# arpitbansal297/Cold-Diffusion-Models

Hardware: AMD Instinct MI355X
Metric: unet_train_imgs_per_sec (higher is better)
Workload: dtype f32 storage/accumulate; dense-conv GEMM operands bf16x3; 1 GPU; CelebA-128 denoising cold diffusion (BASELINE config 3): Unet(dim=64,(1,2,4,8),ch=3) @128x128, T=200, optimizer step = 2 micro-batches x 32 img (one fused forward / backward pass over all of them: same draws, same gradient sum) + Adam + EMA/10; per_gpu_batch=32, gradient_accumulate_every=2, parallelism=single

## Files before the change

cold-diffusion-models_amd/csrc/cdf_common.h:

```cpp
#pragma once
#include <stdint.h>
#include <stddef.h>

#ifdef CDF_EMU
#include "hipemu.h"
#else
#include <hip/hip_runtime.h>
#define CDF_LAUNCH(kernel, grid, block, shmem, stream, ...) \
    hipLaunchKernelGGL(kernel, grid, block, shmem, stream, __VA_ARGS__)
#define CDF_DYN_SMEM(name) extern __shared__ __attribute__((aligned(16))) unsigned char name[]
#define CDF_LDS_BARRIER() asm volatile("s_waitcnt lgkmcnt(0)\n\ts_barrier" ::: "memory")
#define CDF_GLDS16(gptr, lds_base)                                                                            \
    __builtin_amdgcn_global_load_lds((const __attribute__((address_space(1))) void*)(gptr),                    \
                                     (__attribute__((address_space(3))) void*)(lds_base), 16, 0, 0)
#define CDF_WAIT_DMA() asm volatile("s_waitcnt vmcnt(0)" ::: "memory")
#define CDF_WAIT_DMA_LEAVE(N) asm volatile("s_waitcnt vmcnt(%0)" ::"n"(N) : "memory")
#define CDF_SCHED_FENCE() __builtin_amdgcn_sched_barrier(0)
#define CDF_WAIT_LDS() __builtin_amdgcn_s_waitcnt(0xC07F)
typedef float f32x4_t __attribute__((ext_vector_type(4)));
typedef float f32x16_t __attribute__((ext_vector_type(16)));
#endif
#ifndef CDF_EMU
struct CdfDeviceLatch {
    unsigned long long seen = 0;
// ... 78 lines not shown
#ifdef CDF_EMU
struct cdf_buf { const char* base; unsigned bytes; };
static inline cdf_buf cdf_make_buf(const void* p, unsigned bytes) { return cdf_buf{(const char*)p, bytes}; }
static inline float4 cdf_buf_ld(const cdf_buf& b, unsigned off, const float4*) {
    float4 v = make_float4(0.f, 0.f, 0.f, 0.f);
    if ((unsigned long long)off + 16 <= b.bytes) v = *(const float4*)(b.base + off);
    return v;
}
static inline uint2 cdf_buf_ld(const cdf_buf& b, unsigned off, const uint2*) {
    uint2 v = make_uint2(0u, 0u);
    if ((unsigned long long)off + 8 <= b.bytes) v = *(const uint2*)(b.base + off);
    return v;
}
static inline void cdf_buf_st(const cdf_buf& b, unsigned off, const float4& v) {
    if ((unsigned long long)off + 16 <= b.bytes) *(float4*)(b.base + off) = v;
}
static inline void cdf_buf_st(const cdf_buf& b, unsigned off, const uint2& v) {
    if ((unsigned long long)off + 8 <= b.bytes) *(uint2*)(b.base + off) = v;
}
#else
typedef __amdgpu_buffer_rsrc_t cdf_buf;
__device__ __forceinline__ cdf_buf cdf_make_buf(const void* p, unsigned bytes) {
    return __builtin_amdgcn_make_buffer_rsrc((void*)p, 0, (int)bytes, 0x00020000);
}
__device__ __forceinline__ float4 cdf_buf_ld(const cdf_buf& b, unsigned off, const float4*) {
    typedef int i4_t __attribute__((ext_vector_type(4)));
    const i4_t v = __builtin_amdgcn_raw_buffer_load_b128(b, (int)off, 0, 0);
    return make_float4(__int_as_float(v[0]), __int_as_float(v[1]), __int_as_float(v[2]), __int_as_float(v[3]));
}
__device__ __forceinline__ uint2 cdf_buf_ld(const cdf_buf& b, unsigned off, const uint2*) {
    typedef int i2_t __attribute__((ext_vector_type(2)));
    const i2_t v = __builtin_amdgcn_raw_buffer_load_b64(b, (int)off, 0, 0);
    return make_uint2((unsigned)v[0], (unsigned)v[1]);
}
__device__ __forceinline__ void cdf_buf_st(const cdf_buf& b, unsigned off, const float4& v) {
    typedef int i4_t __attribute__((ext_vector_type(4)));
    const i4_t t = {__float_as_int(v.x), __float_as_int(v.y), __float_as_int(v.z), __float_as_int(v.w)};
    __builtin_amdgcn_raw_buffer_store_b128(t, b, (int)off, 0, 0);
}
__device__ __forceinline__ void cdf_buf_st(const cdf_buf& b, unsigned off, const uint2& v) {
    typedef int i2_t __attribute__((ext_vector_type(2)));
    const i2_t t = {(int)v.x, (int)v.y};
    __builtin_amdgcn_raw_buffer_store_b64(t, b, (int)off, 0, 0);
}
#endif
__device__ __forceinline__ float4 cdf_quad_raw(const float4& v, const float4*) { return v; }
__device__ __forceinline__ uint2 cdf_quad_raw(const float4& v, const uint2*) { return make_uint2(cdf_pack2bf(v.x, v.y), cdf_pack2bf(v.z, v.w)); }
__device__ __forceinline__ void cdf_ld4_bf(float* v, const void* base, long long off) {
    const float4 t = cdf_quad_cvt(*(const uint2*)((const unsigned short*)base + off));
    v[0] = t.x; v[1] = t.y; v[2] = t.z; v[3] = t.w;
}
__device__ __forceinline__ void cdf_st4_bf(void* base, long long off, const float* v) {
    uint2 h;
    h.x = cdf_pack2bf(v[0], v[1]);
    h.y = cdf_pack2bf(v[2], v[3]);
    *(uint2*)((unsigned short*)base + off) = h;
}
#define CDF_IO_RES_BF16 1
#define CDF_IO_PRE_BF16 2
#define CDF_IO_MUL_BF16 4
#define CDF_IO_PRE_GRAD 8

#define CDF_OK 0
#define CDF_E_INVALID (-1)
#define CDF_E_UNSUPPORTED (-2)
#define CDF_E_LAUNCH (-3)

#define CDF_WAVE 64
#define CDF_S ((hipStream_t)stream)

void cdf_set_error(const char* fmt, ...);
int cdf_check_launch(const char* what);

#define CDF_REQUIRE(cond, ...)                  \
    do {                                        \
        if (!(cond)) {                          \
            cdf_set_error(__VA_ARGS__);         \
            return CDF_E_INVALID;               \
        }                                       \
    } while (0)

static inline int cdf_cdiv(long long a, long long b) { return (int)((a + b - 1) / b); }

__device__ __forceinline__ int cdf_xcd_order(int bid, int nblk) {
    const int q = nblk >> 3, r = nblk & 7;
    const int xcd = bid & 7, idx = bid >> 3;
    const int base = xcd < r ? xcd * (q + 1) : r * (q + 1) + (xcd - r) * q;
    return base + idx;
}

__device__ __forceinline__ float cdf_wave_sum(float v) {
#pragma unroll
    for (int o = 32; o > 0; o >>= 1) v += __shfl_xor(v, o);
    return v;
}
__device__ __forceinline__ float cdf_wave_max(float v) {
#pragma unroll
    for (int o = 32; o > 0; o >>= 1) v = fmaxf(v, __shfl_xor(v, o));
    return v;
}
__device__ __forceinline__ float cdf_group_sum(float v, int width) {
    for (int o = width >> 1; o > 0; o >>= 1) v += __shfl_xor(v, o);
    return v;
}

__device__ __forceinline__ unsigned cdf_hash32(unsigned long long seed, unsigned long long idx) {
    unsigned long long z = seed + idx * 0x9E3779B97F4A7C15ull;
    z = (z ^ (z >> 30)) * 0xBF58476D1CE4E5B9ull;
    z = (z ^ (z >> 27)) * 0x94D049BB133111EBull;
    z = z ^ (z >> 31);
    return (unsigned)(z >> 32);
}

__device__ __forceinline__ float cdf_erf_fast(float z, float& ez2) {
    const float az = fabsf(z);
#ifdef CDF_EMU
    const float t = 1.0f / fmaf(0.3275911f, az, 1.0f);
    ez2 = expf(-az * az);
#else
    const float t = __builtin_amdgcn_rcpf(fmaf(0.3275911f, az, 1.0f));
    ez2 = __expf(-az * az);
#endif
    float p = fmaf(1.061405429f, t, -1.453152027f);
    p = fmaf(p, t, 1.421413741f);
    p = fmaf(p, t, -0.284496736f);
    p = fmaf(p, t, 0.254829592f);
    const float r = fmaf(-p * t, ez2, 1.0f);
    return copysignf(r, z);
}
__device__ __forceinline__ float cdf_gelu(float x) {
    float e;
    return 0.5f * x * (1.0f + cdf_erf_fast(x * 0.70710678118654752440f, e));
}
__device__ __forceinline__ float cdf_gelu_grad(float x) {
    float e;
    const float cdf = 0.5f * (1.0f + cdf_erf_fast(x * 0.70710678118654752440f, e));
    return cdf + x * (0.39894228040143267794f * e);
}
__device__ __forceinline__ float cdf_gelu_both(float x, float& grad) {
    float e;
    const float er = cdf_erf_fast(x * 0.70710678118654752440f, e);
    const float cdf = 0.5f * (1.0f + er);
    grad = cdf + x * (0.39894228040143267794f * e);
    return 0.5f * x * (1.0f + er);
}
__device__ __forceinline__ float cdf_sigmoid(float x) { return 1.0f / (1.0f + expf(-x)); }
__device__ __forceinline__ float cdf_silu(float x) { return x * cdf_sigmoid(x); }
__device__ __forceinline__ float cdf_silu_grad(float x) {
    const float s = cdf_sigmoid(x);
    return s * (1.0f + x * (1.0f - s));
}
```

cold-diffusion-models_amd/csrc/cdf_conv_sp.h:

```cpp
#pragma once
#include "cdf_common.h"
#include "cdf_epilogue.h"
#include "colddiff.h"

#define CDF_MAX_TAPS 16

typedef short bf16x8_v __attribute__((ext_vector_type(8)));
typedef short bf16x4_v __attribute__((ext_vector_type(4)));
typedef unsigned u32x4_v __attribute__((ext_vector_type(4)));
#ifdef CDF_EMU
#define CDF_MFMA_BF16(a, b, c) __builtin_amdgcn_mfma_f32_32x32x16_bf16(a, b, c, 0, 0, 0)
static inline bf16x4_v cdf_lds_read_tr16(const unsigned short* p) { return hipemu::ds_read_tr16_b64(p); }
#else
typedef __bf16 bf16x8_hw __attribute__((ext_vector_type(8)));
#define CDF_MFMA_BF16(a, b, c) \
    __builtin_amdgcn_mfma_f32_32x32x16_bf16(__builtin_bit_cast(bf16x8_hw, a), __builtin_bit_cast(bf16x8_hw, b), c, 0, 0, 0)
__device__ __forceinline__ bf16x4_v cdf_lds_read_tr16(const unsigned short* p) {
    return __builtin_amdgcn_ds_read_tr16_b64_v4i16((__attribute__((address_space(3))) bf16x4_v*)p);
}
#endif

struct SpPhase {
    int oy, ox, ntaps;
    signed char dy[CDF_MAX_TAPS], dx[CDF_MAX_TAPS], wi[CDF_MAX_TAPS];
// ... 130 lines not shown
        bx = v % gx;
        const int t2 = v / gx;
        by = t2 % gy;
        bz = t2 / gy;
    }
}

#define CDF_GLDS16_K(g, l) CDF_GLDS16(g, l)

struct SpxArgs {
    const unsigned short* x_hi;
    const unsigned short* x_lo;
    const unsigned short* zero;
    const unsigned short* w_hi;
    const unsigned short* w_lo;
    float* y;
    const float* bias;
    const float* sbias;
    const float* res;
    float* pre;
    const float* mul;
    int ldx, ldk, ldy, ld_sbias, ldr, ldp, ldm;
    int B, H, W, Cin, OH, OW, Cout, QH, QW, os, is;
    int act, mul_mode, accumulate, nphase, vec;
    int taprot;
    int dephase;
    unsigned short* ys_hi;
    unsigned short* ys_lo;
    int ld_ys;
    int ksplit;
    float* ks_ws;
    int ks_ld;
    int io_bf;
    int epi;
    const float* ln_x;
    const float* ln_mean;
    const float* ln_rstd;
    float* ln_part;
    int ld_lnx;
    SpPhase ph[4];
};

struct RawEpiArgs {
    int Cout, vec, os, QH, QW, OH, OW, ldy, ldp, ldm, ldr, ld_sbias, ld_ys, act, mul_mode, accumulate, io_bf;
    const float* bias;
    const float* sbias;
    float* pre;
    const float* mul;
    const float* res;
    unsigned short* ys_hi;
    unsigned short* ys_lo;
};

struct SpxWgradArgs {
    const unsigned short* a_hi;
    const unsigned short* a_lo;
    const unsigned short* b_hi;
    const unsigned short* b_lo;
    const unsigned short* zero;
    float* out;
    float* bsum;
    int lda, ldb, ldo;
    int B, QH, QW;
    int HA, WA, sa, HB, WB, sb;
    int CA, CB;
    int ntaps, nsplit, m_per_split, xcd_swizzle;
    signed char day[CDF_MAX_TAPS], dax[CDF_MAX_TAPS], dby[CDF_MAX_TAPS], dbx[CDF_MAX_TAPS];
};

static const cdf_gemm_tuning kTuneDefault = {(int)sizeof(cdf_gemm_tuning), 0, 0, 0, 1, 1, 1, 47, 1, 0, 1, 1, 1, 1, 1, 0, 1};
static inline const cdf_gemm_tuning* cdf_tune(const cdf_gemm_tuning* t) { return (t && t->size == (int)sizeof(cdf_gemm_tuning)) ? t : &kTuneDefault; }
static inline bool cdf_tune_ok(const cdf_gemm_tuning* t) {
    if (!t) return true;
    const bool bm_ok = t->tile_bm == 0 || t->tile_bm == 64 || t->tile_bm == 128 || (t->tile_bm == 256 && (t->tile_bn == 0 || t->tile_bn == 128));
    const bool bn_ok = t->tile_bn == 0 || t->tile_bn == 64 || t->tile_bn == 128;
    return t->size == (int)sizeof(cdf_gemm_tuning) && bm_ok && bn_ok && (t->max_bm == 0 || t->max_bm == 128 || t->max_bm == 256) &&
           (t->halo_bm == 0 || t->halo_bm == 128 || t->halo_bm == 256) && t->halo >= 0 && t->halo <= 127 && t->halo_min_tiles >= 0 && t->resident_reserve >= 0 && t->resident_reserve <= 248 && (t->rowhalo_stream == 0 || t->rowhalo_stream == 1) && (t->epilogue == 0 || t->epilogue == 1);
}
#define CDF_TUNE_CHECK(t, who)                                                                                                          \
    CDF_REQUIRE(cdf_tune_ok(t), who ": bad cdf_gemm_tuning (size %d, expected %d; tile_bm 0/64/128/256 (256 with tile_bn 0/128), tile_bn 0/64/128, " \
                                    "max_bm 0/128/256, halo_bm 0/128/256, halo 0..127, rowhalo_stream 0/1, resident_reserve 0..248, epilogue 0/1): start from cdf_gemm_tuning_default",            \
                (t) ? (t)->size : 0, (int)sizeof(cdf_gemm_tuning))

static inline int cdf_num_cus() {
#ifdef CDF_EMU
    return 8;
#else
    static int n[64] = {0};
    int dev = 0;
    if (hipGetDevice(&dev) != hipSuccess || dev < 0 || dev >= 64) return 256;
    if (!n[dev]) {
        int cus = 0;
        n[dev] = (hipDeviceGetAttribute(&cus, hipDeviceAttributeMultiprocessorCount, dev) == hipSuccess && cus >= 8) ? cus / 8 * 8 : 256;
    }
    return n[dev];
#endif
}


struct CdfPlan {
    int code, tiles, grid;
};
enum { CDF_FORM_ROWHALO = 1, CDF_FORM_HALO = 2, CDF_FORM_SPX = 3, CDF_FORM_WGRAD_ROW3 = 1, CDF_FORM_WGRAD_SPX = 2, CDF_FORM_WGRAD_STACK2 = 3 };
static inline int cdf_plan_set(CdfPlan* p, int form, int bm, int bn, int stages, int ksplit, int w, long long tiles, long long grid) {
    p->code = form << 24 | (bm / 64) << 20 | (bn / 64) << 16 | stages << 12 | ksplit << 4 | (w / 16);
    p->tiles = (int)tiles;
    p->grid = (int)grid;
    return CDF_OK;
}

int cdf_launch_igemm_halo(int ns, int W, bool n64, int bm, const SpxArgs& a, int M, hipStream_t s, CdfPlan* plan = nullptr);
int cdf_launch_igemm_rowhalo(int ns, int W, bool n64, const SpxArgs& a, int M, hipStream_t s, int reserve, CdfPlan* plan = nullptr);
```

cold-diffusion-models_amd/csrc/k_conv.hip:

```cpp
#include <atomic>
#include "cdf_common.h"
#include "cdf_epilogue.h"
#include "colddiff.h"

#define CDF_MAX_TAPS 16

struct ConvPhase {
    int oy, ox, ntaps;
    signed char dy[CDF_MAX_TAPS], dx[CDF_MAX_TAPS], wi[CDF_MAX_TAPS];
};

struct ConvArgs {
    const float* x;
    const float* w;
    float* y;
    const float* bias;
    const float* sbias;
    const float* res;
    float* pre;
    const float* mul;
    int ldx, ldw, ldy, ld_sbias, ldr, ldp, ldm;
    int B, H, W, Cin, OH, OW, Cout, QH, QW, os, is;
    int act;
    int mul_mode;
    int accumulate;
    int nphase, vec;
    unsigned short* ys_hi;
    unsigned short* ys_lo;
    int ld_ys;
    int io_bf;
    long long x_bs, w_bs, y_bs;
    long long x_bs2, w_bs2, y_bs2;
    int epi_follow;
    int batch2;
    ConvPhase ph[4];
};

__device__ __forceinline__ int cdf_xcd_swizzle(int bid, int nblk) {
    const int q = nblk >> 3, r = nblk & 7;
    const int xcd = bid & 7, idx = bid >> 3;
    const int base = xcd < r ? xcd * (q + 1) : r * (q + 1) + (xcd - r) * q;
    return base + idx;
}

template <int BM, int BN, int WM, int WN, bool BT>
__global__ void __launch_bounds__(256, 4) conv_igemm_kernel(ConvArgs a) {
    constexpr int BK = 16, AS = BK + 4;
    constexpr int MT = WM / 32, NT = WN / 32, WAVES_N = BN / WN;
    constexpr int APASS = BM / 64;
    constexpr int BVEC = BK * BN / 4;
    constexpr int BPASS = (BVEC + 255) / 256;
    static_assert((BM / WM) * (BN / WN) == 4, "4 waves per block");
    constexpr int ASZ = BM * AS, BSZ = BK * BN;
    constexpr int EPI_ROWS = (BM / WM) * 32, EPI_SZ = EPI_ROWS * (BN + 8);
    constexpr int SMEM = 2 * (ASZ + BSZ) > EPI_SZ ? 2 * (ASZ + BSZ) : EPI_SZ;
    __shared__ __attribute__((aligned(16))) float smem[SMEM];
    float (*As)[ASZ] = (float (*)[ASZ])smem;
    float (*Bs)[BSZ] = (float (*)[BSZ])(smem + 2 * ASZ);

    const int tid = threadIdx.x, lane = tid & 63, wave = tid >> 6;
    const int wm = wave / WAVES_N, wn = wave % WAVES_N;
    const int M = a.B * a.QH * a.QW;
    const int tiles_n = (a.Cout + BN - 1) / BN, tiles_m = (M + BM - 1) / BM;
    const int tile = cdf_xcd_swizzle(blockIdx.x, tiles_m * tiles_n);
    const int tile_m = tile / tiles_n, tile_n = tile - tile_m * tiles_n;
    const ConvPhase& ph = a.ph[blockIdx.y];
    const int zo = blockIdx.z / a.batch2, zi = blockIdx.z - zo * a.batch2;
    const float* X = a.x + (long long)zo * a.x_bs + (long long)zi * a.x_bs2;
    const float* Wt = a.w + (long long)zo * a.w_bs + (long long)zi * a.w_bs2;
    float* Y = a.y + (long long)zo * a.y_bs + (long long)zi * a.y_bs2;
    long long pix_off = 0;
    if (a.epi_follow) {
        pix_off = ((long long)zo * a.y_bs + (long long)zi * a.y_bs2) / a.ldy;
        Y = a.y;
    }

    const int a_col = (tid & 3) * 4;
    int a_iy0[APASS], a_ix0[APASS];
    unsigned a_pix[APASS];
#pragma unroll
    for (int p = 0; p < APASS; ++p) {
        const int m = tile_m * BM + (tid >> 2) + 64 * p;
        if (m < M) {
            const int qx = m % a.QW, t2 = m / a.QW;
            a_iy0[p] = (t2 % a.QH) * a.is;
            a_ix0[p] = qx * a.is;
            a_pix[p] = (unsigned)(((t2 / a.QH) * a.H + a_iy0[p]) * a.W + a_ix0[p]);
        } else {
            a_iy0[p] = -(1 << 28);
            a_ix0[p] = 0;
            a_pix[p] = 0;
        }
    }
    const int nchunks = (a.Cin + BK - 1) / BK;
    const int niter = ph.ntaps * nchunks;

    __shared__ int tap_lds[CDF_MAX_TAPS + 1];
    if (tid <= CDF_MAX_TAPS)
        tap_lds[tid] = tid < ph.ntaps ? (ph.dy[tid] & 0xFF) | ((ph.dx[tid] & 0xFF) << 8) | ((ph.wi[tid] & 0xFF) << 16) : 0;
    __syncthreads();
    int tap_cur = tap_lds[0];

    f32x4_t ra[APASS], rb[BPASS];
    int tap = 0, c0 = 0, issued = 0;
    auto load_global = [&]() {
        int tc = tap_cur;
#ifndef CDF_EMU
        asm volatile("" : "+v"(tc));
#endif
        const int dy = (int)(signed char)(tc & 0xFF), dx = (int)(signed char)((tc >> 8) & 0xFF), wi = (tc >> 16) & 0xFF;
        const int tap_pix = dy * a.W + dx;
#pragma unroll
        for (int p = 0; p < APASS; ++p) {
            const unsigned iy = (unsigned)(a_iy0[p] + dy), ix = (unsigned)(a_ix0[p] + dx);
            const bool ok = iy < (unsigned)a.H && ix < (unsigned)a.W && (c0 + a_col) < a.Cin;
            const size_t off = (size_t)(a_pix[p] + (unsigned)tap_pix) * (unsigned)a.ldx + (unsigned)(c0 + a_col);
            ra[p] = *(const f32x4_t*)(ok ? X + off : cdf_zero_page);
// ... 16 lines not shown
            }
        }
        const bool more = issued + 1 < niter;
        issued += more ? 1 : 0;
        const int c1 = c0 + BK;
        const bool wrap = c1 >= a.Cin;
        c0 = more ? (wrap ? 0 : c1) : c0;
        tap += (more && wrap) ? 1 : 0;
        tap_cur = tap_lds[tap];
    };
    auto store_lds = [&](int buf) {
#pragma unroll
        for (int p = 0; p < APASS; ++p) *(f32x4_t*)(&As[buf][((tid >> 2) + 64 * p) * AS + a_col]) = ra[p];
#pragma unroll
        for (int p = 0; p < BPASS; ++p) {
            const int idx = tid + 256 * p;
            if (idx < BVEC) {
                if (!BT) {
                    const int k = idx / (BN / 4), n4 = idx - k * (BN / 4);
                    *(f32x4_t*)(&Bs[buf][k * BN + n4 * 4]) = rb[p];
                } else {
                    const int n = idx / (BK / 4), k4 = idx - n * (BK / 4);
                    Bs[buf][(k4 * 4 + 0) * BN + n] = rb[p][0];
                    Bs[buf][(k4 * 4 + 1) * BN + n] = rb[p][1];
                    Bs[buf][(k4 * 4 + 2) * BN + n] = rb[p][2];
                    Bs[buf][(k4 * 4 + 3) * BN + n] = rb[p][3];
                }
            }
        }
    };

    f32x16_t acc[MT][NT];
#pragma unroll
    for (int i = 0; i < MT; ++i)
#pragma unroll
        for (int j = 0; j < NT; ++j)
#pragma unroll
            for (int r = 0; r < 16; ++r) acc[i][j][r] = 0.f;

    const int half = lane >> 5, l31 = lane & 31;
    if (niter > 0) {
        load_global();
        store_lds(0);
    }
    __syncthreads();
    for (int it = 0; it < niter; ++it) {
        const int buf = it & 1;
        load_global();
        float af[MT][8], bf[NT][8];
#pragma unroll
        for (int i = 0; i < MT; ++i) {
            const float* p = &As[buf][(wm * WM + i * 32 + l31) * AS + half * 8];
            const float4 v0 = *(const float4*)p, v1 = *(const float4*)(p + 4);
            af[i][0] = v0.x; af[i][1] = v0.y; af[i][2] = v0.z; af[i][3] = v0.w;
            af[i][4] = v1.x; af[i][5] = v1.y; af[i][6] = v1.z; af[i][7] = v1.w;
        }
#pragma unroll
        for (int j = 0; j < NT; ++j)
#pragma unroll
            for (int s = 0; s < 8; ++s) bf[j][s] = Bs[buf][(half * 8 + s) * BN + wn * WN + j * 32 + l31];
#pragma unroll
        for (int s = 0; s < 8; ++s)
#pragma unroll
            for (int i = 0; i < MT; ++i)
#pragma unroll
                for (int j = 0; j < NT; ++j)
                    acc[i][j] = __builtin_amdgcn_mfma_f32_32x32x2f32(af[i][s], bf[j][s], acc[i][j], 0, 0, 0);
        if (it + 1 < niter) store_lds(buf ^ 1);
        __syncthreads();
    }

    constexpr int CP = BN + 8;
#pragma unroll
    for (int i = 0; i < MT; ++i) {
        if (i > 0) __syncthreads();
#pragma unroll
        for (int j = 0; j < NT; ++j)
#pragma unroll
            for (int r = 0; r < 16; ++r)
                smem[(wm * 32 + (r & 3) + 8 * (r >> 2) + 4 * half) * CP + wn * WN + j * 32 + l31] = acc[i][j][r];
        __syncthreads();
        cdf_epilogue_rows<BN, EPI_ROWS>(a, ph, Y, smem, tile_m * BM, tile_n * BN, M, tid,
                                        [i](int p) { return (p >> 5) * WM + i * 32 + (p & 31); }, pix_off);
    }
}

struct WgradArgs {
    const float* xa;
    const float* xb;
    float* out;
    int lda, ldb, ldo;
    int B, QH, QW;
    int HA, WA, sa, HB, WB, sb;
    int CA, CB;
    int ntaps;
    int nsplit, m_per_split;
    long long a_bs, b_bs, o_bs;
    int nbatch;
    float* bsum;
    signed char day[CDF_MAX_TAPS], dax[CDF_MAX_TAPS], dby[CDF_MAX_TAPS], dbx[CDF_MAX_TAPS];
};

template <int BMC, int BNC, int WM, int WN>
__global__ void __launch_bounds__(256, 4) conv_wgrad_kernel(WgradArgs a) {
    constexpr int BK = 16;
    constexpr int MT = WM / 32, NT = WN / 32, WAVES_N = BNC / WN;
    constexpr int AVEC = BK * BMC / 4, BVEC = BK * BNC / 4;
    constexpr int APASS = (AVEC + 255) / 256, BPASS = (BVEC + 255) / 256;
    static_assert((BMC / WM) * (BNC / WN) == 4, "4 waves per block");
    __shared__ __attribute__((aligned(16))) float Xs[2][BK * BMC];
    __shared__ __attribute__((aligned(16))) float Ys[2][BK * BNC];

    const int tid = threadIdx.x, lane = tid & 63, wave = tid >> 6;
    const int wm = wave / WAVES_N, wn = wave % WAVES_N;
    const int tiles_b = (a.CB + BNC - 1) / BNC;
    int bx = blockIdx.x, by = blockIdx.y, bz = blockIdx.z;
    {
        const int gx = gridDim.x, gy = gridDim.y;
        const int v = cdf_xcd_swizzle(bx + gx * (by + gy * bz), gx * gy * (int)gridDim.z);
        bx = v % gx;
        const int t2 = v / gx;
        by = t2 % gy;
        bz = t2 / gy;
    }
    const int tile_a = bx / tiles_b, tile_b = bx - tile_a * tiles_b;
    const int tap = by;
    const int batch = bz / a.nsplit, split = bz - batch * a.nsplit;
    const float* XA = a.xa + (long long)batch * a.a_bs;
    const float* XB = a.xb + (long long)batch * a.b_bs;
    const int M = a.B * a.QH * a.QW;
    const int m_lo = split * a.m_per_split;
    int m_hi = m_lo + a.m_per_split;
    if (m_hi > M) m_hi = M;
    const int niter = m_hi > m_lo ? (m_hi - m_lo + BK - 1) / BK : 0;
    const int day = a.day[tap], dax = a.dax[tap], dby = a.dby[tap], dbx = a.dbx[tap];

    int a_q[APASS][3], b_q[BPASS][3];
    auto decode = [&](int m, int* q) {
        q[0] = m % a.QW;
        const int t2 = m / a.QW;
        q[1] = t2 % a.QH;
        q[2] = t2 / a.QH;
    };
    auto advance = [&](int* q) {
        q[0] += BK;
        while (q[0] >= a.QW) {
            q[0] -= a.QW;
            if (++q[1] >= a.QH) { q[1] = 0; ++q[2]; }
        }
    };
#pragma unroll
    for (int p = 0; p < APASS; ++p) decode(m_lo + (tid + 256 * p) / (BMC / 4), a_q[p]);
#pragma unroll
    for (int p = 0; p < BPASS; ++p) decode(m_lo + (tid + 256 * p) / (BNC / 4), b_q[p]);
    const bool do_bsum = a.bsum != nullptr && tile_a == 0 && tap == 0;
    float4 bs_acc[BPASS];
#pragma unroll
    for (int p = 0; p < BPASS; ++p) bs_acc[p] = make_float4(0.f, 0.f, 0.f, 0.f);

    float4 ra[APASS], rb[BPASS];
    auto load_global = [&](int it) {
        const int m0 = m_lo + it * BK;
#pragma unroll
        for (int p = 0; p < APASS; ++p) {
            const int idx = tid + 256 * p;
            ra[p] = make_float4(0.f, 0.f, 0.f, 0.f);
// ... 230 lines not shown
        for (int k = 0; k < NE; ++k) tot[k] += old[k];
    }
#pragma unroll
    for (int k = 0; k < NE; ++k)
        if (ok[k]) *dst[k] = tot[k];
}

template <int T_, int RJ>
__global__ void __launch_bounds__(256) unpack_reduce_tiled_kernel(const float* ws, float* g, int nsplit, int R, int C, int ldc, long long s_t,
                                                                   long long s_r, long long s_c, int accumulate, const float* bws, float* gb,
                                                                   int bC, int bld, int order) {
    __shared__ float red[8 * T_ * RJ * 33 > 8 * 33 ? 8 * T_ * RJ * 33 : 8 * 33];
    if (blockIdx.y == 1) {
        if ((int)blockIdx.x < (bC + 31) / 32) unpack_tile_body<1, 1>(bws, gb, nsplit, 1, bC, bld, 0, 0, 1, accumulate, blockIdx.x, red, 1);
        return;
    }
    unpack_tile_body<T_, RJ>(ws, g, nsplit, R, C, ldc, s_t, s_r, s_c, accumulate, blockIdx.x, red, order);
}

template <bool BF>
__global__ void colsum_partial_kernel(const void* xv, float* part, int rows_per_seg, int rows_per_chunk, int C, int ld) {
    typedef typename cdf_quad<BF>::elem elem_t;
    const elem_t* x = (const elem_t*)xv;
    __shared__ float red[4][64];
    const int c = blockIdx.x * 64 + (threadIdx.x & 63), rl = threadIdx.x >> 6;
    const int r0 = blockIdx.z * rows_per_chunk;
    int r1 = r0 + rows_per_chunk;
    if (r1 > rows_per_seg) r1 = rows_per_seg;
    const elem_t* p = x + (long long)blockIdx.y * rows_per_seg * ld;
    float s = 0.f;
    if (c < C) {
        elem_t t[8];
        int r = r0 + rl;
        for (; r + 28 < r1; r += 32) {
#pragma unroll
            for (int u = 0; u < 8; ++u) t[u] = p[(long long)(r + 4 * u) * ld + c];
            s += ((cdf_widen(t[0]) + cdf_widen(t[1])) + (cdf_widen(t[2]) + cdf_widen(t[3]))) +
                 ((cdf_widen(t[4]) + cdf_widen(t[5])) + (cdf_widen(t[6]) + cdf_widen(t[7])));
        }
        for (; r < r1; r += 4) s += cdf_widen(p[(long long)r * ld + c]);
    }
    red[rl][threadIdx.x & 63] = s;
    __syncthreads();
    if (rl == 0 && c < C) {
        const int l = threadIdx.x;
        part[((long long)blockIdx.y * gridDim.z + blockIdx.z) * C + c] = (red[0][l] + red[1][l]) + (red[2][l] + red[3][l]);
    }
}
__global__ void __launch_bounds__(1024) colsum_final_kernel(const float* part, float* out, int nchunk, int C, int ldo, int accumulate) {
    __shared__ float red[16][64];
    const int l = threadIdx.x & 63, rl = threadIdx.x >> 6, c = blockIdx.x * 64 + l;
    float s = 0.f;
    if (c < C) {
        const float* p = part + (long long)blockIdx.y * nchunk * C + c;
        for (int k = rl; k < nchunk; k += 16) s += p[(long long)k * C];
    }
    red[rl][l] = s;
    __syncthreads();
    if (rl == 0 && c < C) {
        float t = 0.f;
#pragma unroll
        for (int r = 0; r < 16; ++r) t += red[r][l];
        float* dst = out + (long long)blockIdx.y * ldo + c;
        *dst = accumulate ? *dst + t : t;
    }
}

static int check_feat(const char* who, const void* p, int ld, int C) {
    CDF_REQUIRE(p != nullptr, "%s: null tensor", who);
    CDF_REQUIRE((((uintptr_t)p) & 15) == 0, "%s: tensor not 16-byte aligned", who);
    CDF_REQUIRE(ld % 4 == 0 && ld >= C, "%s: pitch %d must be a multiple of 4 and >= C=%d", who, ld, C);
    return CDF_OK;
}

template <int BM, int BN, int WM, int WN>
static int launch_conv(const ConvArgs& a, int batch, bool bt, hipStream_t s) {
    const int M = a.B * a.QH * a.QW;
    const int tiles = cdf_cdiv(M, BM) * cdf_cdiv(a.Cout, BN);
    if (bt)
        CDF_LAUNCH((conv_igemm_kernel<BM, BN, WM, WN, true>), dim3(tiles, a.nphase, batch), dim3(256), 0, s, a);
    else
        CDF_LAUNCH((conv_igemm_kernel<BM, BN, WM, WN, false>), dim3(tiles, a.nphase, batch), dim3(256), 0, s, a);
    return cdf_check_launch("conv_igemm");
}

extern "C" int cdf_conv_gemm_io(const float* x, int ldx, const float* w, int ldw, float* y, int ldy, int B, int H, int W,
                                int Cin, int OH, int OW, int Cout, int QH, int QW, int os, int is, int nphase,
                                const int* phase_desc, const float* bias, const float* sbias, int ld_sbias,
                                const void* res, int ldr, void* pre, int ldp, const void* mul, int ldm, int act,
                                int mul_mode, int accumulate, int b_trans, int batch, long long x_bs, long long w_bs,
                                long long y_bs, int batch2, long long x_bs2, long long w_bs2, long long y_bs2, int io_bf16, void* y_hi,
                                int ld_ys, void* stream);

extern "C" int cdf_conv_gemm(const float* x, int ldx, const float* w, int ldw, float* y, int ldy, int B, int H, int W,
                             int Cin, int OH, int OW, int Cout, int QH, int QW, int os, int is, int nphase,
                             const int* phase_desc, const float* bias, const float* sbias, int ld_sbias,
                             const float* res, int ldr, float* pre, int ldp, const float* mul, int ldm, int act,
                             int mul_mode, int accumulate, int b_trans, int batch, long long x_bs, long long w_bs,
                             long long y_bs, int batch2, long long x_bs2, long long w_bs2, long long y_bs2, void* stream) {
    return cdf_conv_gemm_io(x, ldx, w, ldw, y, ldy, B, H, W, Cin, OH, OW, Cout, QH, QW, os, is, nphase, phase_desc, bias, sbias, ld_sbias, res, ldr,
                            pre, ldp, mul, ldm, act, mul_mode, accumulate, b_trans, batch, x_bs, w_bs, y_bs, batch2, x_bs2, w_bs2, y_bs2, 0, nullptr, 0,
                            stream);
}

extern "C" int cdf_conv_gemm_io(const float* x, int ldx, const float* w, int ldw, float* y, int ldy, int B, int H, int W,
                                int Cin, int OH, int OW, int Cout, int QH, int QW, int os, int is, int nphase,
                                const int* phase_desc, const float* bias, const float* sbias, int ld_sbias,
                                const void* res_, int ldr, void* pre_, int ldp, const void* mul_, int ldm, int act,
                                int mul_mode, int accumulate, int b_trans, int batch, long long x_bs, long long w_bs,
                                long long y_bs, int batch2, long long x_bs2, long long w_bs2, long long y_bs2, int io_bf16, void* y_hi,
                                int ld_ys, void* stream) {
    const float* res = (const float*)res_;
    float* pre = (float*)pre_;
    const float* mul = (const float*)mul_;
    int rc;
    CDF_REQUIRE((io_bf16 & ~7) == 0, "cdf_conv_gemm_io: io_bf16 has unknown bits (%d)", io_bf16);
    CDF_REQUIRE(y || (y_hi && !accumulate), "cdf_conv_gemm_io: no output (y NULL needs y_hi and no accumulate)");
    CDF_REQUIRE(!y_hi || (ld_ys % 4 == 0 && ld_ys >= Cout && Cout % 4 == 0 && (((uintptr_t)y_hi) & 7) == 0), "cdf_conv_gemm_io: the output plane needs Cout %% 4 == 0, ld_ys %% 4 == 0, 8-byte alignment");
    if ((rc = check_feat("cdf_conv_gemm(x)", x, ldx, Cin))) return rc;
    if (y && (rc = check_feat("cdf_conv_gemm(y)", y, 4, 0))) return rc;
    CDF_REQUIRE(w && (((uintptr_t)w) & 15) == 0 && ldw % 4 == 0, "cdf_conv_gemm: weights must be 16B aligned, ldw%%4==0");
    CDF_REQUIRE(ldy >= Cout, "cdf_conv_gemm: ldy < Cout");
    CDF_REQUIRE(nphase >= 1 && nphase <= 4 && phase_desc, "cdf_conv_gemm: nphase must be 1..4");
    CDF_REQUIRE(B > 0 && H > 0 && W > 0 && Cin > 0 && Cout > 0 && QH > 0 && QW > 0 && batch >= 1 && batch2 >= 1, "cdf_conv_gemm: bad shape");
    CDF_REQUIRE(!b_trans || (Cin % 4 == 0), "cdf_conv_gemm: b_trans needs K %% 4 == 0");
    CDF_REQUIRE(!mul_mode || mul, "cdf_conv_gemm: mul_mode without mul tensor");
    ConvArgs a;
    a.x = x; a.w = w; a.y = y; a.bias = bias; a.sbias = sbias; a.res = res; a.pre = pre; a.mul = mul;
    a.ldx = ldx; a.ldw = ldw; a.ldy = ldy; a.ld_sbias = ld_sbias; a.ldr = ldr; a.ldp = ldp; a.ldm = ldm;
    a.B = B; a.H = H; a.W = W; a.Cin = Cin; a.OH = OH; a.OW = OW; a.Cout = Cout; a.QH = QH; a.QW = QW;
    a.os = os; a.is = is; a.act = act; a.mul_mode = mul_mode; a.accumulate = accumulate; a.nphase = nphase;
    a.x_bs = x_bs; a.w_bs = w_bs; a.y_bs = y_bs;
    a.x_bs2 = x_bs2; a.w_bs2 = w_bs2; a.y_bs2 = y_bs2; a.batch2 = batch2;
    a.vec = cdf_epi_vec_ok(Cout, y, ldy, bias, sbias, ld_sbias, res, ldr, pre, ldp, mul, ldm) && y_bs % 4 == 0 && y_bs2 % 4 == 0;
    a.epi_follow = 0;
    if ((long long)batch * batch2 > 1 && (res || pre || mul)) {
        CDF_REQUIRE(y_bs % ldy == 0 && y_bs2 % ldy == 0 && !sbias, "cdf_conv_gemm: batched launches with pre / mul / res operands need per-batch outputs that are whole rows "
                    "of y (y_bs and y_bs2 multiples of ldy) and no per-sample bias");
        a.epi_follow = 1;
    }
    a.ys_hi = (unsigned short*)y_hi; a.ys_lo = nullptr; a.ld_ys = ld_ys; a.io_bf = io_bf16;
    CDF_REQUIRE((!y_hi && !io_bf16) || a.vec, "cdf_conv_gemm_io: bf16 operands / the output plane need the vectorised epilogue (16-byte-aligned pointers, pitches %% 4, Cout %% 4)");
    CDF_REQUIRE(y || (long long)batch * batch2 == 1 || a.epi_follow, "cdf_conv_gemm_io: a batched launch without y needs an epilogue operand (row-offset addressing)");
    batch *= batch2;
    const int* pd = phase_desc;
    for (int p = 0; p < nphase; ++p) {
        a.ph[p].oy = pd[0]; a.ph[p].ox = pd[1]; a.ph[p].ntaps = pd[2];
        CDF_REQUIRE(pd[2] >= 0 && pd[2] <= CDF_MAX_TAPS, "cdf_conv_gemm: too many taps (%d)", pd[2]);
        for (int t = 0; t < pd[2]; ++t) {
            a.ph[p].dy[t] = (signed char)pd[3 + 3 * t];
            a.ph[p].dx[t] = (signed char)pd[4 + 3 * t];
            a.ph[p].wi[t] = (signed char)pd[5 + 3 * t];
        }
        pd += 3 + 3 * pd[2];
    }
    const bool bt = b_trans != 0;
    if (Cout <= 32) return launch_conv<128, 32, 32, 32>(a, batch, bt, CDF_S);
    if (Cout <= 64) return launch_conv<256, 64, 64, 64>(a, batch, bt, CDF_S);
    return launch_conv<128, 128, 64, 64>(a, batch, bt, CDF_S);
}

template <int BMC, int BNC, int WM, int WN>
static int launch_wgrad(const WgradArgs& a, int batch, hipStream_t s) {
    const int tiles = cdf_cdiv(a.CA, BMC) * cdf_cdiv(a.CB, BNC);
    CDF_LAUNCH((conv_wgrad_kernel<BMC, BNC, WM, WN>), dim3(tiles, a.ntaps, batch * a.nsplit), dim3(256), 0, s, a);
    return cdf_check_launch("conv_wgrad");
}

extern "C" int cdf_wgrad_nsplit(int M, int CA, int CB, int ntaps) {
    auto tiles_of = [&](int c) { return c <= 64 ? 1 : cdf_cdiv(c, 128); };
    const int tiles = tiles_of(CA) * tiles_of(CB) * ntaps;
    int ns = 1024 / tiles;
    const int max_by_m = M / 256 > 0 ? M / 256 : 1;
    if (ns > max_by_m) ns = max_by_m;
    if (ns < 1) ns = 1;
    if (ns > 256) ns = 256;
    return ns;
}

extern "C" int cdf_conv_wgrad(const float* xa, int lda, const float* xb, int ldb, float* ws, int ldo, int B, int QH,
                              int QW, int HA, int WA, int sa, int HB, int WB, int sb, int CA, int CB, int ntaps,
                              const int* tap_desc, int nsplit, int batch, long long a_bs, long long b_bs,
                              long long o_bs, float* bsum, void* stream) {
    int rc;
    if ((rc = check_feat("cdf_conv_wgrad(xa)", xa, lda, CA))) return rc;
    if ((rc = check_feat("cdf_conv_wgrad(xb)", xb, ldb, CB))) return rc;
    CDF_REQUIRE(ws && ldo % 4 == 0 && ldo >= CB, "cdf_conv_wgrad: bad workspace pitch");
    CDF_REQUIRE(ntaps >= 1 && ntaps <= CDF_MAX_TAPS && tap_desc, "cdf_conv_wgrad: bad tap count");
    CDF_REQUIRE(nsplit >= 1 && batch >= 1, "cdf_conv_wgrad: bad split/batch");
    WgradArgs a;
    a.xa = xa; a.xb = xb; a.out = ws; a.lda = lda; a.ldb = ldb; a.ldo = ldo;
    a.B = B; a.QH = QH; a.QW = QW; a.HA = HA; a.WA = WA; a.sa = sa; a.HB = HB; a.WB = WB; a.sb = sb;
    a.CA = CA; a.CB = CB; a.ntaps = ntaps; a.nsplit = nsplit;
    const int M = B * QH * QW;
    a.m_per_split = cdf_cdiv(cdf_cdiv(M, nsplit), 16) * 16;
    a.a_bs = a_bs; a.b_bs = b_bs; a.o_bs = o_bs; a.bsum = bsum; a.nbatch = batch;
    for (int t = 0; t < ntaps; ++t) {
        a.day[t] = (signed char)tap_desc[4 * t + 0];
        a.dax[t] = (signed char)tap_desc[4 * t + 1];
        a.dby[t] = (signed char)tap_desc[4 * t + 2];
        a.dbx[t] = (signed char)tap_desc[4 * t + 3];
    }
    if (CA <= 32) {
        if (CB <= 32) return launch_wgrad<64, 64, 32, 32>(a, batch, CDF_S);
        return launch_wgrad<32, 128, 32, 32>(a, batch, CDF_S);
    }
    if (CB <= 32) return launch_wgrad<128, 32, 32, 32>(a, batch, CDF_S);
    if (CA <= 64 && CB <= 64) return launch_wgrad<64, 64, 32, 32>(a, batch, CDF_S);
    if (CA <= 64) return launch_wgrad<64, 128, 32, 64>(a, batch, CDF_S);
    if (CB <= 64) return launch_wgrad<128, 64, 64, 32>(a, batch, CDF_S);
    return launch_wgrad<128, 128, 64, 64>(a, batch, CDF_S);
}

static inline int ew_grid2(long long n) {
    long long g = (n + 255) / 256;
    if (g > 4096) g = 4096;
    return g < 1 ? 1 : (int)g;
}

struct CdfPackEntry {
    const float* src;
    void* dst0;
    void* dst1;
    long long s_t, s_r, s_c;
    int T, R, C, ldc, kind, first_block;
};

__global__ void __launch_bounds__(256) pack_many_kernel(const CdfPackEntry* tab, int nentries) {
    int lo = 0, hi = nentries - 1;
    const int b = blockIdx.x;
    while (lo < hi) {
        const int mid = (lo + hi + 1) >> 1;
        if (tab[mid].first_block <= b) lo = mid; else hi = mid - 1;
    }
    const CdfPackEntry e = tab[lo];
    if (e.s_t == 1 && e.T > 1 && e.T <= 16) {
        const long long n2 = (long long)e.R * e.ldc;
        const long long j0 = (long long)(b - e.first_block) * 1024 + threadIdx.x;
        const long long plane = (long long)e.R * e.ldc;
// ... 127 lines not shown
```

Measured before the change: 1259 img/s.

## Add persistent streaming 1x1 conv kernel that keeps weight panel resident in LDS

Adds a conv_stream_kernel for 1x1 stride-1 convolutions with Cin up to 128. Each block loads the full weight panel into LDS once, then walks a run of M tiles and prefetches the next tile's activations into registers while running f32 MFMA on the current one. The run length is sized from CU count and LDS occupancy, and cdf_num_cus moves to the common header so it can be used here. The aim is to cut repeated weight loads and per-tile launch overhead on small-K pointwise convs, at the cost of fewer blocks and the slower f32 MFMA path instead of bf16.

```diff
diff --git a/cold-diffusion-models_amd/csrc/cdf_common.h b/cold-diffusion-models_amd/csrc/cdf_common.h
--- a/cold-diffusion-models_amd/csrc/cdf_common.h
+++ b/cold-diffusion-models_amd/csrc/cdf_common.h
@@ -184,6 +184,21 @@
 
 static inline int cdf_cdiv(long long a, long long b) { return (int)((a + b - 1) / b); }
 
+static inline int cdf_num_cus() {
+#ifdef CDF_EMU
+    return 8;
+#else
+    static int n[64] = {0};
+    int dev = 0;
+    if (hipGetDevice(&dev) != hipSuccess || dev < 0 || dev >= 64) return 256;
+    if (!n[dev]) {
+        int cus = 0;
+        n[dev] = (hipDeviceGetAttribute(&cus, hipDeviceAttributeMultiprocessorCount, dev) == hipSuccess && cus >= 8) ? cus / 8 * 8 : 256;
+    }
+    return n[dev];
+#endif
+}
+
 __device__ __forceinline__ int cdf_xcd_order(int bid, int nblk) {
     const int q = nblk >> 3, r = nblk & 7;
     const int xcd = bid & 7, idx = bid >> 3;
diff --git a/cold-diffusion-models_amd/csrc/cdf_conv_sp.h b/cold-diffusion-models_amd/csrc/cdf_conv_sp.h
--- a/cold-diffusion-models_amd/csrc/cdf_conv_sp.h
+++ b/cold-diffusion-models_amd/csrc/cdf_conv_sp.h
@@ -236,20 +236,6 @@
                                     "max_bm 0/128/256, halo_bm 0/128/256, halo 0..127, rowhalo_stream 0/1, resident_reserve 0..248, epilogue 0/1): start from cdf_gemm_tuning_default",            \
                 (t) ? (t)->size : 0, (int)sizeof(cdf_gemm_tuning))
 
-static inline int cdf_num_cus() {
-#ifdef CDF_EMU
-    return 8;
-#else
-    static int n[64] = {0};
-    int dev = 0;
-    if (hipGetDevice(&dev) != hipSuccess || dev < 0 || dev >= 64) return 256;
-    if (!n[dev]) {
-        int cus = 0;
-        n[dev] = (hipDeviceGetAttribute(&cus, hipDeviceAttributeMultiprocessorCount, dev) == hipSuccess && cus >= 8) ? cus / 8 * 8 : 256;
-    }
-    return n[dev];
-#endif
-}
 
 
 struct CdfPlan {
diff --git a/cold-diffusion-models_amd/csrc/k_conv.hip b/cold-diffusion-models_amd/csrc/k_conv.hip
--- a/cold-diffusion-models_amd/csrc/k_conv.hip
+++ b/cold-diffusion-models_amd/csrc/k_conv.hip
@@ -33,6 +33,8 @@
     long long x_bs2, w_bs2, y_bs2;
     int epi_follow;
     int batch2;
+    int epi;
+    int st_tpb;
     ConvPhase ph[4];
 };
 
@@ -215,6 +217,145 @@
         __syncthreads();
         cdf_epilogue_rows<BN, EPI_ROWS>(a, ph, Y, smem, tile_m * BM, tile_n * BN, M, tid,
                                         [i](int p) { return (p >> 5) * WM + i * 32 + (p & 31); }, pix_off);
+    }
+}
+
+constexpr int CDF_STREAM_MAX_CIN = 128;
+
+template <int NCH, int BN, bool BT>
+__global__ void __launch_bounds__(256) conv_stream_kernel(ConvArgs a) {
+    constexpr int NT = BN / 32, KP = NCH * 16, CP = BN + 8, BM = 128;
+    constexpr int BVEC = KP * BN / 4, BPASS = BVEC / 256;
+    constexpr int GC = KP < 64 ? KP : 64, NG = KP / GC, CPG = GC / 16, LPR = GC / 4, RPI = 64 / LPR, IPG = 32 / RPI;
+    constexpr int AS = GC + 4;
+    constexpr int WSZ = 32 * (AS > CP ? AS : CP);
+    static_assert(BVEC % 256 == 0 && (BN == 32 || BN == 64), "B panel divides among the threads");
+    __shared__ __attribute__((aligned(16))) float Bs[KP * BN];
+    __shared__ __attribute__((aligned(16))) float wlds[4 * WSZ];
+
+    const int tid = threadIdx.x, lane = tid & 63, wave = tid >> 6, half = lane >> 5, l31 = lane & 31;
+    const int M = a.B * a.QH * a.QW;
+    const int tiles_n = (a.Cout + BN - 1) / BN, tiles_m = (M + BM - 1) / BM;
+    const int v = cdf_xcd_swizzle(blockIdx.x, gridDim.x);
+    const int run = v / tiles_n, tile_n = v - run * tiles_n;
+    const int t_lo = run * a.st_tpb;
+    const int t_hi = t_lo + a.st_tpb < tiles_m ? t_lo + a.st_tpb : tiles_m;
+    const ConvPhase& ph = a.ph[0];
+    const int zo = blockIdx.z / a.batch2, zi = blockIdx.z - zo * a.batch2;
+    const float* X = a.x + (long long)zo * a.x_bs + (long long)zi * a.x_bs2;
+    const float* Wt = a.w + (long long)zo * a.w_bs + (long long)zi * a.w_bs2;
+    float* Y = a.y ? a.y + (long long)zo * a.y_bs + (long long)zi * a.y_bs2 : nullptr;
+    long long pix_off = 0;
+    if (a.epi_follow) {
+        pix_off = ((long long)zo * a.y_bs + (long long)zi * a.y_bs2) / a.ldy;
+        Y = a.y;
+    }
+    const int n_base = tile_n * BN;
+
+    f32x4_t rb[BPASS];
+#pragma unroll
+    for (int p = 0; p < BPASS; ++p) {
+        const int idx = tid + 256 * p;
+        if (!BT) {
+            const int k = idx / (BN / 4), n4 = idx - k * (BN / 4);
+            const int co = n_base + n4 * 4;
+            const bool ok = k < a.Cin && co < a.Cout;
+            rb[p] = *(const f32x4_t*)(ok ? Wt + (size_t)(unsigned)k * (unsigned)a.ldw + (unsigned)co : cdf_zero_page);
+        } else {
+            const int n = idx / (KP / 4), k4 = idx - n * (KP / 4);
+            const int ci = k4 * 4, co = n_base + n;
+            const bool ok = ci < a.Cin && co < a.Cout;
+            rb[p] = *(const f32x4_t*)(ok ? Wt + (size_t)(unsigned)co * (unsigned)a.ldw + (unsigned)ci : cdf_zero_page);
+        }
+    }
+
+    const int a_row = lane / LPR, a_c4 = (lane % LPR) * 4;
+    f32x4_t ra[NG][IPG];
+    auto load_group = [&](int t, int g) {
+        const int ch = g * GC + a_c4;
+        const int m0 = t * BM + wave * 32 + a_row;
+        const bool cok = t < t_hi && ch < a.Cin;
+        const float* base = X + (size_t)(unsigned)m0 * (unsigned)a.ldx + ch;
+#pragma unroll
+        for (int i = 0; i < IPG; ++i)
+            ra[g][i] = *(const f32x4_t*)((cok && m0 + RPI * i < M) ? base + (size_t)(RPI * i) * (unsigned)a.ldx : cdf_zero_page);
+    };
+#pragma unroll
+    for (int g = 0; g < NG; ++g) load_group(t_lo, g);
+
+#pragma unroll
+    for (int p = 0; p < BPASS; ++p) {
+        const int idx = tid + 256 * p;
+        if (!BT) {
+            *(f32x4_t*)(&Bs[idx * 4]) = rb[p];
+        } else {
+            const int n = idx / (KP / 4), k4 = idx - n * (KP / 4);
+#pragma unroll
+            for (int e = 0; e < 4; ++e) Bs[(k4 * 4 + e) * BN + n] = rb[p][e];
+        }
+    }
+    CDF_LDS_BARRIER();
+
+    float* wl = wlds + wave * WSZ;
+    for (int t = t_lo; t < t_hi; ++t) {
+        f32x16_t acc[NT];
+#pragma unroll
+        for (int j = 0; j < NT; ++j)
+#pragma unroll
+            for (int r = 0; r < 16; ++r) acc[j][r] = 0.f;
+#pragma unroll
+        for (int g = 0; g < NG; ++g) {
+            CDF_WAVE_SYNC();
+#pragma unroll
+            for (int i = 0; i < IPG; ++i) *(f32x4_t*)(wl + (RPI * i + a_row) * AS + a_c4) = ra[g][i];
+            load_group(t + 1, g);
+            CDF_WAVE_SYNC();
+#pragma unroll
+            for (int cc = 0; cc < CPG; ++cc) {
+                const int c = g * CPG + cc;
+                const float* fp = wl + l31 * AS + cc * 16 + half * 8;
+                const f32x4_t v0 = *(const f32x4_t*)fp, v1 = *(const f32x4_t*)(fp + 4);
+                const float af[8] = {v0[0], v0[1], v0[2], v0[3], v1[0], v1[1], v1[2], v1[3]};
+                float bf[NT][8];
+#pragma unroll
+                for (int j = 0; j < NT; ++j)
+#pragma unroll
+                    for (int s = 0; s < 8; ++s) bf[j][s] = Bs[(c * 16 + half * 8 + s) * BN + j * 32 + l31];
+#pragma unroll
+                for (int s = 0; s < 8; ++s)
+#pragma unroll
+                    for (int j = 0; j < NT; ++j) acc[j] = __builtin_amdgcn_mfma_f32_32x32x2f32(af[s], bf[j][s], acc[j], 0, 0, 0);
+            }
+        }
+
+        const int m_base = t * BM + wave * 32;
+        if (m_base >= M) continue;
+        auto dump = [&]() {
+            CDF_WAVE_SYNC();
+#pragma unroll
+            for (int j = 0; j < NT; ++j)
+#pragma unroll
+                for (int r = 0; r < 16; ++r) wl[((r & 3) + 8 * (r >> 2) + 4 * half) * CP + j * 32 + l31] = acc[j][r];
+            CDF_WAVE_SYNC();
+        };
+        if (cdf_epi_tile_ok<32, BN>(a, M)) {
+            const long long row0 = m_base + pix_off;
+            ConvArgs b = a;
+            b.y = Y;
+            auto body = [&](auto spec) {
+                using E = cdf_epi_fast<BN, 32, 64, decltype(spec)>;
+                f32x4_t q[E::NR], bs[2];
+                cdf_epi_load_bias<BN, 64>(b, bs, row0, n_base, lane);
+                E::load(b, q, row0, n_base, lane);
+                dump();
+                E::finish(b, q, bs, wl, row0, n_base, lane);
+            };
+            if (a.epi >= 7) cdf_epi_dispatch<true>(a.epi, body);
+            else cdf_epi_dispatch<false>(a.epi, body);
+        } else {
+            dump();
+            cdf_epilogue_rows<BN, 32, 64>(a, ph, Y, wl, m_base, n_base, M, lane, [](int p) { return p; }, pix_off);
+        }
     }
 }
 
@@ -611,6 +752,32 @@
     else
         CDF_LAUNCH((conv_igemm_kernel<BM, BN, WM, WN, false>), dim3(tiles, a.nphase, batch), dim3(256), 0, s, a);
     return cdf_check_launch("conv_igemm");
+}
+
+static bool conv_stream_eligible(const ConvArgs& a) {
+    return a.nphase == 1 && a.ph[0].ntaps == 1 && a.ph[0].dy[0] == 0 && a.ph[0].dx[0] == 0 && a.ph[0].wi[0] == 0 && a.is == 1 &&
+           a.QH == a.H && a.QW == a.W && a.Cin <= CDF_STREAM_MAX_CIN;
+}
+
+template <int NCH, int BN>
+static int launch_conv_stream(ConvArgs& a, int batch, bool bt, hipStream_t s) {
+    const int M = a.B * a.QH * a.QW;
+    const int tiles_m = cdf_cdiv(M, 128), tiles_n = cdf_cdiv(a.Cout, BN);
+    const int as = (NCH * 16 < 64 ? NCH * 16 : 64) + 4, cp = BN + 8;
+    const int lds = (NCH * 16 * BN + 4 * 32 * (as > cp ? as : cp)) * (int)sizeof(float);
+    const int per_cu = 160 * 1024 / lds < 4 ? 160 * 1024 / lds : 4;
+    long long runs = (long long)cdf_num_cus() * per_cu / ((long long)tiles_n * batch);
+    if (runs < 1) runs = 1;
+    if (runs > tiles_m) runs = tiles_m;
+    int tpb = cdf_cdiv(tiles_m, runs);
+    if (tpb < 2 && tiles_m >= 2) tpb = 2;
+    a.st_tpb = tpb;
+    const dim3 grid(cdf_cdiv(tiles_m, tpb) * tiles_n, 1, batch);
+    if (bt)
+        CDF_LAUNCH((conv_stream_kernel<NCH, BN, true>), grid, dim3(256), 0, s, a);
+    else
+        CDF_LAUNCH((conv_stream_kernel<NCH, BN, false>), grid, dim3(256), 0, s, a);
+    return cdf_check_launch("conv_stream");
 }
 
 extern "C" int cdf_conv_gemm_io(const float* x, int ldx, const float* w, int ldw, float* y, int ldy, int B, int H, int W,
@@ -684,6 +851,18 @@
         pd += 3 + 3 * pd[2];
     }
     const bool bt = b_trans != 0;
+    a.epi = cdf_epi_select(a);
+    a.st_tpb = 0;
+    if (conv_stream_eligible(a)) {
+        if (Cout <= 32) {
+            if (Cin <= 32) return launch_conv_stream<2, 32>(a, batch, bt, CDF_S);
+            if (Cin <= 64) return launch_conv_stream<4, 32>(a, batch, bt, CDF_S);
+        } else {
+            if (Cin <= 32) return launch_conv_stream<2, 64>(a, batch, bt, CDF_S);
+            if (Cin <= 64) return launch_conv_stream<4, 64>(a, batch, bt, CDF_S);
+            return launch_conv_stream<8, 64>(a, batch, bt, CDF_S);
+        }
+    }
     if (Cout <= 32) return launch_conv<128, 32, 32, 32>(a, batch, bt, CDF_S);
     if (Cout <= 64) return launch_conv<256, 64, 64, 64>(a, batch, bt, CDF_S);
     return launch_conv<128, 128, 64, 64>(a, batch, bt, CDF_S);
```

New measurement: 1261 img/s, median of 6. About the same (+0.2%).
